# vladiant/CascadeClassifier

Measured on AMD Instinct MI355X. Metric: detection Mwindows/sec (1080p, haarcascade_frontalface) + achieved HBM GB/s, higher is better.
Workload: dtype i32+f32 (f64 stage sums)

## Files before the change

### cascadeclassifier_amd/csrc/cc_eval_kernel.inc

```

#define CC_CONST __attribute__((address_space(4)))
template <class T>
__device__ __forceinline__ const T CC_CONST* as_const_table(const T* p) {
  return (const T CC_CONST*)p;
}
template <class T>
__device__ __forceinline__ T load_record(const T CC_CONST* p) {
  static_assert(sizeof(T) % 4 == 0, "table records are dword multiples");
  T out;
  const int CC_CONST* w = (const int CC_CONST*)p;
  int* o = reinterpret_cast<int*>(&out);
#pragma unroll
  for (unsigned i = 0; i < sizeof(T) / 4; i++) o[i] = w[i];
  return out;
}

constexpr int STAGE_ROWS = 12;
template <int STEP, class Geom>
__device__ __forceinline__ void stage_tile(int32_t* lds, const Geom& G, const int32_t* __restrict__ sum,
                                           const ScaleDev& S, int x0, int y0) {
  const int lane = threadIdx.x & 63, wave = __builtin_amdgcn_readfirstlane(threadIdx.x >> 6);
  const int quads = (G.cols + 3) >> 2;
  const bool right_edge = x0 + quads * 4 - 1 > S.w;
  for (int q0 = 0; q0 < quads; q0 += 64) {
// ... 67 lines not shown
  int sq_compact;
  int split_stumps;
  int stop_after;
  unsigned long long* masks;
  size_t mask_frame_words;
  CandRaw* cands;
  int* cand_count;
  int cand_cap;
  int32_t* dbg_codes;
  double* dbg_sums;
  unsigned long long* stamps;
};
constexpr int STAMP_SLOTS = 40;

struct LdsReader {
  const int32_t* b;
  __device__ __forceinline__ int operator()(int ofs) const { return b[ofs]; }
};
struct GlobalReader {
  const int32_t* g;
  unsigned org;
  int pitch;
  __device__ __forceinline__ int operator()(int p) const { return g[org + (unsigned)((p >> 16) * pitch + (p & 0xffff))]; }
};
template <class R>
__device__ __forceinline__ double stump_vote(const R& rd, const HaarStumpDev& sp, float vnf) {
  const int r0 = rd(sp.ofs[0][0]) - rd(sp.ofs[0][1]) - rd(sp.ofs[0][2]) + rd(sp.ofs[0][3]);
  const int r1 = rd(sp.ofs[1][0]) - rd(sp.ofs[1][1]) - rd(sp.ofs[1][2]) + rd(sp.ofs[1][3]);
  float v = sp.w[0] * (float)r0 + sp.w[1] * (float)r1;
  if (sp.nrect == 3) {
    const int r2 = rd(sp.ofs[2][0]) - rd(sp.ofs[2][1]) - rd(sp.ofs[2][2]) + rd(sp.ofs[2][3]);
    v += sp.w[2] * (float)r2;
  }
  v *= vnf;
  return (double)(v < sp.thr ? sp.left : sp.right);
}
template <class R>
__device__ __forceinline__ double stump_vote(const R& rd, const HaarStumpDev CC_CONST* spp, float vnf) {
  return stump_vote(rd, load_record(spp), vnf);
}

struct Lds16Reader {
  const unsigned short* h;
  __device__ __forceinline__ int operator()(int ofs) const { return (int)h[ofs]; }
};
template <bool M16, class R>
__device__ __forceinline__ float lbp_vote_f(const R& rd, const LbpStumpDev& sp) {
  int p[16];
#pragma unroll
  for (int j = 0; j < 16; j++) p[j] = rd(sp.ofs[j]);
  auto cell = [&](int a, int b, int c2, int d) {
    const int v = p[a] - p[b] - p[c2] + p[d];
    return M16 ? (v & 0xffff) : v;
  };
  const int c = cell(5, 6, 9, 10);
  const bool b7 = cell(0, 1, 4, 5) >= c, b6 = cell(1, 2, 5, 6) >= c, b5 = cell(2, 3, 6, 7) >= c;
  const int lo = (cell(6, 7, 10, 11) >= c ? 16 : 0) | (cell(10, 11, 14, 15) >= c ? 8 : 0) | (cell(9, 10, 13, 14) >= c ? 4 : 0) |
                 (cell(8, 9, 12, 13) >= c ? 2 : 0) | (cell(4, 5, 8, 9) >= c ? 1 : 0);
  const int l0 = b5 ? sp.subset[1] : sp.subset[0], l1 = b5 ? sp.subset[3] : sp.subset[2], l2 = b5 ? sp.subset[5] : sp.subset[4],
            l3 = b5 ? sp.subset[7] : sp.subset[6];
  const int m0 = b6 ? l1 : l0, m1 = b6 ? l3 : l2;
  const unsigned w = (unsigned)(b7 ? m1 : m0);
  return ((w >> lo) & 1u) ? sp.left : sp.right;
}

template <class R>
__device__ __forceinline__ double stump_vote(const R& rd, const LbpStumpDev CC_CONST* sp, float) {
  int p[16];
#pragma unroll
  for (int j = 0; j < 16; j++) p[j] = rd(sp->ofs[j]);
  const int c = p[5] - p[6] - p[9] + p[10];
  const int lbp = (p[0] - p[1] - p[4] + p[5] >= c ? 128 : 0) | (p[1] - p[2] - p[5] + p[6] >= c ? 64 : 0) |
                  (p[2] - p[3] - p[6] + p[7] >= c ? 32 : 0) | (p[6] - p[7] - p[10] + p[11] >= c ? 16 : 0) |
                  (p[10] - p[11] - p[14] + p[15] >= c ? 8 : 0) | (p[9] - p[10] - p[13] + p[14] >= c ? 4 : 0) |
                  (p[8] - p[9] - p[12] + p[13] >= c ? 2 : 0) | (p[4] - p[5] - p[8] + p[9] >= c ? 1 : 0);
  const int word = sp->subset[lbp >> 5];
  return (double)((word & (1 << (lbp & 31))) ? sp->left : sp->right);
}

__device__ __forceinline__ double tree_vote(const int32_t* b, const HaarNodeDev* __restrict__ nodes, int root, int leaf0,
                                            const float* __restrict__ leaves, float vnf) {
  int idx = 0;
  do {
    const HaarNodeDev* n = nodes + root + idx;
    const int r0 = b[n->ofs[0][0]] - b[n->ofs[0][1]] - b[n->ofs[0][2]] + b[n->ofs[0][3]];
    const int r1 = b[n->ofs[1][0]] - b[n->ofs[1][1]] - b[n->ofs[1][2]] + b[n->ofs[1][3]];
    float v = n->w[0] * (float)r0 + n->w[1] * (float)r1;
    if (n->nrect == 3) v += n->w[2] * (float)(b[n->ofs[2][0]] - b[n->ofs[2][1]] - b[n->ofs[2][2]] + b[n->ofs[2][3]]);
    v *= vnf;
    idx = v < n->thr ? n->left : n->right;
  } while (idx > 0);
  return (double)leaves[leaf0 - idx];
}
__device__ __forceinline__ double tree_vote(const int32_t* b, const LbpNodeDev* __restrict__ nodes, int root, int leaf0,
                                            const float* __restrict__ leaves, float) {
  int idx = 0;
  do {
    const LbpNodeDev* n = nodes + root + idx;
    int p[16];
#pragma unroll
    for (int j = 0; j < 16; j++) p[j] = b[n->ofs[j]];
    const int c = p[5] - p[6] - p[9] + p[10];
    const int lbp = (p[0] - p[1] - p[4] + p[5] >= c ? 128 : 0) | (p[1] - p[2] - p[5] + p[6] >= c ? 64 : 0) |
                    (p[2] - p[3] - p[6] + p[7] >= c ? 32 : 0) | (p[6] - p[7] - p[10] + p[11] >= c ? 16 : 0) |
                    (p[10] - p[11] - p[14] + p[15] >= c ? 8 : 0) | (p[9] - p[10] - p[13] + p[14] >= c ? 4 : 0) |
                    (p[8] - p[9] - p[12] + p[13] >= c ? 2 : 0) | (p[4] - p[5] - p[8] + p[9] >= c ? 1 : 0);
    idx = (n->subset[lbp >> 5] & (1 << (lbp & 31))) ? n->left : n->right;
  } while (idx > 0);
  return (double)leaves[leaf0 - idx];
}

template <int CTRL, int ROW_MASK>
__device__ __forceinline__ int dpp_i32(int v) {
  return __builtin_amdgcn_update_dpp(0, v, CTRL, ROW_MASK, 0xF, false);
}
__device__ __forceinline__ int wave_max_u32(int v) {
  v = max(v, dpp_i32<0xB1, 0xF>(v));
  v = max(v, dpp_i32<0x4E, 0xF>(v));
  v = max(v, dpp_i32<0x141, 0xF>(v));
  v = max(v, dpp_i32<0x140, 0xF>(v));
  v = max(v, dpp_i32<0x142, 0xA>(v));
  v = max(v, dpp_i32<0x143, 0xC>(v));
  return __builtin_amdgcn_readlane(v, 63);
}
__device__ __forceinline__ int wave_sum_u32(int v) {
  v += dpp_i32<0xB1, 0xF>(v);
  v += dpp_i32<0x4E, 0xF>(v);
  v += dpp_i32<0x141, 0xF>(v);
  v += dpp_i32<0x140, 0xF>(v);
  v += dpp_i32<0x142, 0xA>(v);
  v += dpp_i32<0x143, 0xC>(v);
  return __builtin_amdgcn_readlane(v, 63);
}

__device__ __forceinline__ float inv_sqrt_as_float(double nf) {
#ifndef CC_EXACT_SLOW_VNF
  double y = __builtin_amdgcn_rsq(nf);
#pragma unroll
  for (int it = 0; it < 2; it++) {
    const double e = __builtin_fma(-(nf * y), y, 1.0);
    y = __builtin_fma(0.5 * y, e, y);
  }
  const unsigned below = (unsigned)(unsigned long long)__double_as_longlong(y) & 0x1fffffffu;
  if (__builtin_expect(below - 0x0ffffc00u > 0x800u, 1)) return (float)y;
#endif
  return (float)(1. / sqrt(nf));
}

#ifdef CC_SPEC_STAGES
template <int STEP>
__device__ __forceinline__ double spec_stage(int st, int p_lo, int p_hi, const int32_t* b, float vnf);
template <int STEP>
__device__ __forceinline__ void spec_stage0_x2(const int32_t* ba, const int32_t* bb, float vnfa, float vnfb, double& acc_a, double& acc_b);
#endif

template <bool C, class A, class B>
struct cc_select {
  using type = A;
};
template <class A, class B>
struct cc_select<false, A, B> {
  using type = B;
};

template <int STEP, bool HAAR, bool TREES>
__device__ __forceinline__ void eval_tile(const EvalArgs& A, int32_t* lds, const int4 T, const ScaleDev& S) {
  using Stump = typename cc_select<HAAR, HaarStumpDev, LbpStumpDev>::type;
  using Node = typename cc_select<HAAR, HaarNodeDev, LbpNodeDev>::type;
  const Node* __restrict__ nodes = reinterpret_cast<const Node*>(STEP == 2 ? A.nodes2 : A.nodes1);
#ifdef CC_SPEC_W0
  constexpr int W0 = CC_SPEC_W0, H0 = CC_SPEC_H0;
#else
  const int W0 = A.W0, H0 = A.H0;
#endif
#ifdef CC_SPEC_TILE16
  constexpr bool G16 = STEP == 2 && !TREES;
#else
  constexpr bool G16 = false;
#endif
  using Geom = typename cc_select<G16, TileGeom16, TileGeom<STEP>>::type;
  const Geom G(W0, H0);
  double* s_part = reinterpret_cast<double*>(lds + tile_words_padded(G.words()) * ((HAAR && A.tilt_chan >= 0) ? 2 : 1));
  float* s_vnf = reinterpret_cast<float*>(s_part + PART_DOUBLES);
  unsigned short* s_q = reinterpret_cast<unsigned short*>(s_vnf + (HAAR ? TILE_Y * VNF_PITCH : 0));
  int* s_cnt = reinterpret_cast<int*>(s_q + 2 * TILE_WINDOWS);
  const int frame = blockIdx.y;
  const int32_t* sum = A.integ + ((size_t)frame * A.nchan + 0) * A.int_frame_elems + S.int_ofs;
  const int lane = threadIdx.x & 63, wave = __builtin_amdgcn_readfirstlane(threadIdx.x >> 6);
  const int gx0 = T.y * TILE_X, gy0 = T.z * TILE_Y;
  const Stump CC_CONST* stumps = as_const_table(reinterpret_cast<const Stump*>(G16 ? A.gstumps : STEP == 2 ? A.stumps2 : A.stumps1));
  const int CC_CONST* stage_first = as_const_table(A.stage_first);
  const int CC_CONST* stage_ntrees = as_const_table(A.stage_ntrees);
  const float CC_CONST* stage_thr = as_const_table(A.stage_thr);
  const bool dbg = A.dbg_codes != nullptr && frame == 0;
  auto stamp = [&](int slot) {
    if (A.stamps && threadIdx.x == 0)
      A.stamps[((size_t)blockIdx.y * gridDim.x + blockIdx.x) * STAMP_SLOTS + slot] = __builtin_amdgcn_s_memtime();
  };
  stamp(0);

  unsigned sq_raw[WIN_PER_THREAD][4];
#pragma unroll
  for (int k = 0; k < WIN_PER_THREAD; k++) {
    sq_raw[k][0] = sq_raw[k][1] = sq_raw[k][2] = sq_raw[k][3] = 0;
    if (HAAR) {
      const int gx = min(gx0 + lane, S.nx - 1), gy = min(gy0 + wave * WIN_PER_THREAD + k, S.ny - 1);
      {
        const unsigned* sq = reinterpret_cast<const unsigned*>(A.integ + ((size_t)frame * A.nchan + 1) * A.int_frame_elems + S.int_ofs);
        const int nrx = W0 - 2, nry = H0 - 2;
        size_t q0;
        int dx;
        if (STEP == 2 && A.sq_compact) {
          q0 = (size_t)(gy * 2 + 1) * S.pitchI + gx;
          dx = nrx >> 1;
        } else {
          q0 = (size_t)(gy * STEP + 1) * S.pitchI + (gx * STEP + 1);
          dx = nrx;
        }
        sq_raw[k][0] = sq[q0];
        sq_raw[k][1] = sq[q0 + dx];
        sq_raw[k][2] = sq[q0 + (size_t)nry * S.pitchI];
        sq_raw[k][3] = sq[q0 + (size_t)nry * S.pitchI + dx];
      }
    }
  }
#ifdef CC_PRIO_STAGE
  __builtin_amdgcn_s_setprio(CC_PRIO_STAGE);
#endif
  stage_tile<STEP>(lds, G, sum, S, gx0 * STEP, gy0 * STEP);
  if (HAAR && A.tilt_chan >= 0)
    stage_tile<STEP>(lds + tile_words_padded(G.words()), G,
                     A.integ + ((size_t)frame * A.nchan + A.tilt_chan) * A.int_frame_elems + S.int_ofs, S, gx0 * STEP, gy0 * STEP);
  if (threadIdx.x < 3 * 32) s_cnt[threadIdx.x] = 0;
  unsigned valsq_pre[WIN_PER_THREAD];
#pragma unroll
  for (int k = 0; k < WIN_PER_THREAD; k++) valsq_pre[k] = sq_raw[k][0] - sq_raw[k][1] - sq_raw[k][2] + sq_raw[k][3];
  __syncthreads();
#ifdef CC_PRIO_STAGE
  __builtin_amdgcn_s_setprio(0);
#endif
  stamp(1);

  if (A.stop_after == -2) return;
  auto window_base = [&](int id) { return ((id >> 6) * STEP) * G.row_stride + (id & 63); };
  auto table_reader = [&](int id) {
    if constexpr (G16)
      return GlobalReader{sum, (unsigned)((gy0 + (id >> 6)) * STEP) * (unsigned)S.pitchI + (unsigned)((gx0 + (id & 63)) * STEP), S.pitchI};
    else
      return LdsReader{lds + window_base(id)};
  };
  auto report = [&](int id, int code, double last) {
    const size_t o = (size_t)S.win_ofs + (size_t)(gy0 + (id >> 6)) * S.nx + (gx0 + (id & 63));
    A.dbg_codes[o] = code;
    if (A.dbg_sums) A.dbg_sums[o] = last;
  };
  auto emit_candidate = [&](int id, double last_sum) {
    const int slot = atomicAdd(A.cand_count, 1);
    if (slot < A.cand_cap) A.cands[slot] = CandRaw{frame, T.x, gx0 + (id & 63), gy0 + (id >> 6), last_sum};
  };
  const int skew = (STEP * G.row_stride) & 31;
  auto win_class = [&](int id) { return ((id & 63) + skew * (id >> 6)) & 31; };
  auto vnf_slot = [&](int id) { return (id >> 6) * (TILE_X + skew) + (id & 63); };
  auto enqueue = [&](bool pass, int id, int g) {
    if (g >= A.dense_from) {
      const unsigned long long m = __ballot(pass);
      int first = 0;
      if (lane == 0 && m) first = atomicAdd(&s_cnt[(g % 3) * 32], __builtin_popcountll(m));
      first = __builtin_amdgcn_readfirstlane(first);
      if (pass) s_q[(g & 1) * TILE_WINDOWS + first + __builtin_amdgcn_mbcnt_hi((unsigned)(m >> 32), __builtin_amdgcn_mbcnt_lo((unsigned)m, 0))] = (unsigned short)id;
    } else if (pass) {
      const int c = win_class(id);
      const int row = atomicAdd(&s_cnt[(g % 3) * 32 + c], 1);
      s_q[(g & 1) * TILE_WINDOWS + row * 32 + c] = (unsigned short)id;
    }
  };

  const int CC_CONST* group_first = as_const_table(A.group_first);
  auto stage_sum = [&](int s, int id, const int32_t* b, float vnf, bool want) -> double {
    double acc = 0.;
    const int first = stage_first[s], nt = stage_ntrees[s];
    if constexpr (TREES) {
      for (int j = 0; j < nt; j++) {
        const int root = as_const_table(A.tree_root)[first + j], leaf0 = as_const_table(A.tree_leaf0)[first + j];
        if (want) acc += tree_vote(b, nodes, root, leaf0, A.leaves, vnf);
      }
    } else {
#ifdef CC_SPEC_STAGES
      if (s < CC_SPEC_STAGES) return spec_stage<STEP>(s, 0, SPEC_PARTS, b, vnf);
#endif
      const auto rd = table_reader(id);
      if constexpr (HAAR) {
        Stump cur = load_record(stumps + first);
        for (int j = 0; j < nt; j++) {
          const Stump nxt = load_record(stumps + first + min(j + 1, nt - 1));
          acc += stump_vote(rd, cur, vnf);
          cur = nxt;
        }
      } else {
        for (int j = 0; j < nt; j++) acc += stump_vote(rd, stumps + first + j, vnf);
      }
    }
    return acc;
  };

  if constexpr (!HAAR && !TREES && WIN_PER_THREAD > 2) {
    const int gx = gx0 + lane;
    const double thr0 = (double)stage_thr[0];
    const int nt0 = stage_ntrees[0];
#pragma unroll 1
    for (int k = 0; k < WIN_PER_THREAD; k++) {
      const int ly = wave * WIN_PER_THREAD + k;
      const int gy = gy0 + ly;
      const int id = ly * 64 + lane;
      const int32_t* b = lds + (ly * STEP) * G.row_stride + lane;
      const bool alive = gx < S.nx && gy < S.ny;
      double acc = 0.;
      if (__any(alive)) {
#ifdef CC_SPEC_STAGES
        acc = spec_stage<STEP>(0, 0, SPEC_PARTS, b, 1.f);
#else
        for (int i = 0; i < nt0; i++) acc += stump_vote(LdsReader{b}, stumps + i, 1.f);
#endif
      }
      (void)nt0;
      bool pass = alive && !(acc < thr0);
      const bool rej0 = alive && !pass;
      const unsigned long long m = __ballot(rej0);
      if (lane == 0 && gy < S.ny) A.masks[(size_t)frame * A.mask_frame_words + S.mask_ofs + (size_t)gy * S.nxw + T.y] = m;
      if (dbg && rej0) report(id, 0, acc);
      if (!dbg && A.early_skip) {
        const unsigned long long lower = (1ull << lane) - 1ull;
        const unsigned long long zeros_below = ~m & lower;
        int run;
        bool known;
        if (zeros_below) {
          run = lane - 1 - (63 - __clzll((long long)zeros_below));
          known = true;
        } else {
          run = lane;
          known = T.y == 0;
        }
        if (known && (run & 1)) pass = false;
      }
      if (A.nstages == 1) {
        if (pass) {
          emit_candidate(id, acc);
          if (dbg) report(id, 1, acc);
        }
      } else
        enqueue(pass, id, 1);
    }
  } else {
    int base[WIN_PER_THREAD];
    float vnf[WIN_PER_THREAD];
    bool alive[WIN_PER_THREAD];
    const int gx = gx0 + lane;
#pragma unroll
    for (int k = 0; k < WIN_PER_THREAD; k++) {
      const int ly = wave * WIN_PER_THREAD + k;
      const int gy = gy0 + ly;
      base[k] = (ly * STEP) * G.row_stride + lane;
      vnf[k] = 1.f;
      alive[k] = gx < S.nx && gy < S.ny;
      if (HAAR) {
        const bool in_grid = alive[k];
        alive[k] = false;
        if (in_grid) {
          const int nrx = W0 - 2, nry = H0 - 2;
          const double area = (double)(nrx * nry);
          const int32_t* b = lds + base[k];
          int valsum;
          if constexpr (G16) {
            const unsigned short* h = reinterpret_cast<const unsigned short*>(b);
            const int hx = nrx >> 1;
            const unsigned a0 = h[G.at(1, 1)], a1 = h[G.at(1, 1 + hx)], a2 = h[G.at(1, 1 + nrx)];
            const unsigned c0 = h[G.at(1 + nry, 1)], c1 = h[G.at(1 + nry, 1 + hx)], c2 = h[G.at(1 + nry, 1 + nrx)];
            valsum = (int)(((a0 - a1 - c0 + c1) & 0xffffu) + ((a1 - a2 - c1 + c2) & 0xffffu));
          } else
            valsum = b[G.at(1, 1)] - b[G.at(1, 1 + nrx)] - b[G.at(1 + nry, 1)] + b[G.at(1 + nry, 1 + nrx)];
          const unsigned valsq = valsq_pre[k];
          double nf = area * (double)valsq - (double)valsum * (double)valsum;
          if (nf > 0.) {
            vnf[k] = inv_sqrt_as_float(nf);
            alive[k] = area * (double)vnf[k] < 1e-1;
          }
          if (dbg && !alive[k]) report(ly * 64 + lane, -1, 0.0);
        }
      }
    }
    if (A.stop_after == -3) {
      float sink = 0;
#pragma unroll
      for (int k = 0; k < WIN_PER_THREAD; k++) sink += alive[k] ? vnf[k] : 0.f;
      if (HAAR && sink == 12345.f) s_vnf[0] = sink;
      return;
    }
    bool any_mine = false;
    double acc[WIN_PER_THREAD];
#pragma unroll
    for (int k = 0; k < WIN_PER_THREAD; k++) {
      any_mine |= alive[k];
      acc[k] = 0.;
    }
    if (__any(any_mine)) {
      const int nt = stage_ntrees[0];
      if constexpr (TREES) {
        for (int i = 0; i < nt; i++) {
          const int root = as_const_table(A.tree_root)[i], leaf0 = as_const_table(A.tree_leaf0)[i];
#pragma unroll
          for (int k = 0; k < WIN_PER_THREAD; k++)
            if (alive[k]) acc[k] += tree_vote(lds + base[k], nodes, root, leaf0, A.leaves, vnf[k]);
        }
      } else if constexpr (HAAR) {
#ifdef CC_SPEC_STAGES
        if constexpr (WIN_PER_THREAD == 2) {
          spec_stage0_x2<STEP>(lds + base[0], lds + base[1], vnf[0], vnf[1], acc[0], acc[1]);
        } else {
#pragma unroll
          for (int k = 0; k < WIN_PER_THREAD; k++) acc[k] = spec_stage<STEP>(0, 0, SPEC_PARTS, lds + base[k], vnf[k]);
        }
#else
        Stump cur = load_record(stumps);
        for (int i = 0; i < nt; i++) {
          const Stump nxt = load_record(stumps + min(i + 1, nt - 1));
#pragma unroll
          for (int k = 0; k < WIN_PER_THREAD; k++) acc[k] += stump_vote(LdsReader{lds + base[k]}, cur, vnf[k]);
          cur = nxt;
        }
#endif
      } else {
#ifdef CC_SPEC_STAGES
        if constexpr (WIN_PER_THREAD == 2) {
          spec_stage0_x2<STEP>(lds + base[0], lds + base[1], vnf[0], vnf[1], acc[0], acc[1]);
        } else {
#pragma unroll
          for (int k = 0; k < WIN_PER_THREAD; k++) acc[k] = spec_stage<STEP>(0, 0, SPEC_PARTS, lds + base[k], vnf[k]);
        }
#else
        for (int i = 0; i < nt; i++) {
#pragma unroll
          for (int k = 0; k < WIN_PER_THREAD; k++) acc[k] += stump_vote(LdsReader{lds + base[k]}, stumps + i, vnf[k]);
        }
#endif
      }
    }
    const double thr = (double)stage_thr[0];
    bool pass_k[WIN_PER_THREAD];
#pragma unroll
    for (int k = 0; k < WIN_PER_THREAD; k++) {
      const int ly = wave * WIN_PER_THREAD + k;
      const int gy = gy0 + ly;
      const int id = ly * 64 + lane;
      bool pass = alive[k] && !(acc[k] < thr);
      const bool rej0 = alive[k] && !pass;
      const unsigned long long m = __ballot(rej0);
      if (lane == 0 && gy < S.ny) A.masks[(size_t)frame * A.mask_frame_words + S.mask_ofs + (size_t)gy * S.nxw + T.y] = m;
      if (dbg && rej0) report(id, 0, acc[k]);
      if (!dbg && A.early_skip) {
        const unsigned long long lower = (1ull << lane) - 1ull;
        const unsigned long long zeros_below = ~m & lower;
        int run;
        bool known;
        if (zeros_below) {
          run = lane - 1 - (63 - __clzll((long long)zeros_below));
          known = true;
        } else {
          run = lane;
          known = T.y == 0;
        }
        if (known && (run & 1)) pass = false;
      }
      pass_k[k] = pass;
    }
#pragma unroll
    for (int k = 0; k < WIN_PER_THREAD; k++) {
      const int id = (wave * WIN_PER_THREAD + k) * 64 + lane;
      const bool pass = pass_k[k];
      if (A.nstages == 1) {
        if (pass) {
          emit_candidate(id, acc[k]);
          if (dbg) report(id, 1, acc[k]);
        }
      } else {
        if (HAAR && pass) s_vnf[vnf_slot(id)] = vnf[k];
        enqueue(pass, id, 1);
      }
    }
  }

  stamp(2);
#ifdef CC_PRIO_LATE
  __builtin_amdgcn_s_setprio(CC_PRIO_LATE);
#endif
  const int half = lane >> 5, cls = lane & 31;
  int st = 1;
  int qg = 1;
  int n = 0, rows = 0, my_rows = 0;
  for (; qg < A.ngroups; qg++) {
    st = group_first[qg];
    const int st_end = group_first[qg + 1];
    if (A.stop_after >= 0 && st > A.stop_after) return;
    __syncthreads();
    if (qg >= A.dense_from) {
      n = min(s_cnt[(qg % 3) * 32], TILE_WINDOWS);
// ... 288 lines not shown
```

### cascadeclassifier_amd/csrc/cc_spec.hip

```cpp
#include <hip/hip_runtime.h>

#include <algorithm>
#include <array>
#include <cmath>
#include <cstdlib>
#include <cstring>
#include <map>
#include <mutex>

#include <dlfcn.h>
#include <sys/stat.h>
#include <unistd.h>

#include "cc_detect_internal.h"

namespace ccamd {

#include "build/cc_eval_kernel_src.h"

struct SpecStump {
  std::string loads;
  std::string decls;
  std::string compute;
  double base = 0.;
  long long base_q = 0;
};

static const char* spec_stage_inline_attr() {
  const char* e = std::getenv("CCAMD_SPEC_NOINLINE");
  return (e && std::atoi(e) != 0) ? "__noinline__" : "__forceinline__";
}

static void spec_emit_stage(std::string& o, const std::vector<SpecStump>& st, int depth, bool parts, const std::vector<std::string>& accs,
                            bool fixed_point = false) {
  const int nt = (int)st.size();
  static const char* kSB = "      __builtin_amdgcn_sched_barrier(0);\n";
  for (const SpecStump& t : st) o += "      " + t.decls + "\n";
  const int P = parts ? SPEC_PARTS : 1;
  char buf[128];
  int prev_nonempty = -1;
  for (int k = 0; k < P; k++) {
    const int e0 = (int)((long long)k * nt / P), e1 = (int)((long long)(k + 1) * nt / P);
    if (e0 == e1) continue;
    if (parts)
      snprintf(buf, sizeof(buf), "      if (p_lo > %d && p_lo <= %d) {\n", prev_nonempty, k);
    else
      snprintf(buf, sizeof(buf), "      {\n");
    prev_nonempty = k;
    o += buf;
    for (int i = e0; i < std::min(e0 + depth, nt); i++) o += "      " + st[(size_t)i].loads + "\n" + kSB;
    o += "      }\n";
    if (parts) {
      snprintf(buf, sizeof(buf), "      if (p_lo <= %d && %d < p_hi) {\n", k, k);
      o += buf;
    } else
      o += "      {\n";
    {
      double base = 0.;
      unsigned base_q = 0;
      for (int i = e0; i < e1; i++) {
        base += st[(size_t)i].base;
        base_q += (unsigned)st[(size_t)i].base_q;
      }
      char lit[64];
      if (fixed_point)
        snprintf(lit, sizeof(lit), "%uu", base_q);
      else
        snprintf(lit, sizeof(lit), "%a", base);
      if (fixed_point ? base_q != 0 : base != 0.)
        for (const std::string& a : accs) o += "      " + a + " += " + lit + ";\n";
    }
    for (int i = e0; i < e1; i++) {
      if (depth > 0 && i + depth < nt) o += "      " + st[(size_t)(i + depth)].loads + "\n" + kSB;
      if (depth == 0) o += "      " + st[(size_t)i].loads + "\n";
      o += "      " + st[(size_t)i].compute + "\n" + kSB;
    }
    o += "      }\n";
  }
}

static std::string spec_stage_source_lbp(const Cascade& m, int n_stages, bool tile16);

static std::vector<std::array<int, 4>> pieces16(int x, int y, int w, int h) {
  std::vector<std::array<int, 4>> out;
  const bool along_x = w >= h;
  const int len = along_x ? w : h;
  for (int k = 1; k <= std::max(len, 1); k++) {
    out.clear();
    bool ok = true;
    for (int i = 0; i < k; i++) {
      const int a = (int)((long long)i * len / k), b = (int)((long long)(i + 1) * len / k);
      if (a == b) continue;
      const std::array<int, 4> pc = along_x ? std::array<int, 4>{x + a, y, b - a, h} : std::array<int, 4>{x, y + a, w, b - a};
      ok = ok && fits16((long long)pc[2] * pc[3]);
      out.push_back(pc);
    }
    if (ok) return out;
  }
  return {};
}

static bool tile16_eligible(const Cascade& m, int n_stages) {
  if (m.max_nodes_per_tree > 1) return false;
  const int total = (int)m.stage_ntrees.size();
  n_stages = std::min<int>(n_stages, total);
  const char* on = std::getenv("CCAMD_SPEC_TILE16");
  if (on ? std::atoi(on) == 0 : !(m.feature_type == CC_FEATURE_LBP && n_stages == total)) return false;
  if (m.feature_type == CC_FEATURE_HAAR) {
    if (m.has_tilted) return false;
    const int nrx = m.win_w - 2, nry = m.win_h - 2;
    if (nrx < 2 || !fits16((long long)(nrx - (nrx >> 1)) * nry)) return false;
    if (!fits16(std::max(m.win_w, m.win_h))) return false;
    return true;
  }
  for (int s = 0; s < n_stages; s++)
    for (int i = 0; i < m.stage_ntrees[(size_t)s]; i++) {
      const int32_t* r = &m.lbp_rects[(size_t)m.stump_feature[(size_t)m.stage_first[(size_t)s] + i] * 4];
      if (!fits16((long long)r[2] * r[3])) return false;
    }
  return true;
}

static std::string spec_stage_source(const Cascade& m, int n_stages, int tmode) {
  const CNumericLocale c_numbers;
  if (m.feature_type == CC_FEATURE_LBP) return spec_stage_source_lbp(m, n_stages, tmode == TILE_16);
  std::vector<HaarStumpDev> t[2];
  build_haar_stumps<1>(m, t[0]);
  build_haar_stumps<2>(m, t[1]);
  const TileGeom16 G16(m.win_w, m.win_h);
  n_stages = std::min<int>(n_stages, (int)m.stage_ntrees.size());
  const int depth = 2;
  const bool delta_form = stage_sums_order_independent(m, 4.0);
  std::string o;
  char buf[512];
  auto hexf = [&](float v) {
    snprintf(buf, sizeof(buf), "%af", (double)v);
    return std::string(buf);
  };
  auto stage_quantum = [&](int s, double& q) {
    int emin = INT32_MAX;
    double mag = 0;
    for (int i = 0; i < m.stage_ntrees[(size_t)s]; i++) {
      const size_t k = (size_t)m.stage_first[(size_t)s] + i;
      const float l = m.stump_left[k], r = m.stump_right[k];
      mag += std::max(std::fabs((double)l), std::fabs((double)r));
      for (float v : {l, r})
        if (v != 0.0f) {
          int e;
          std::frexp(v, &e);
          emin = std::min(emin, e);
        }
    }
    if (emin == INT32_MAX) return false;
    q = std::ldexp(1.0, emin - 24);
    return mag / q < 2147483647.0;
  };
  std::function<std::string(const HaarStumpDev&, const std::string&, double, SpecStump&)> vote_text;
  auto stump = [&](const HaarStumpDev& d, int stump_index, int local, const std::string& win, double fixed_q, bool h16,
                   const std::map<int, std::string>* reuse = nullptr, std::map<int, std::string>* vars_out = nullptr) {
    const int fi = m.stump_feature[(size_t)stump_index];
    const std::string tile_ptr = (h16 ? "h" : "b") + win;
    bool int_ok = true;
    double bound = 0;
    for (int j = 0; j < d.nrect; j++) {
      const float w = d.w[j];
      const int32_t* r = &m.haar_rects[(size_t)fi * 12 + j * 4];
      if (w != std::nearbyint(w) || std::fabs(w) > 64.f) int_ok = false;
      bound += std::fabs((double)w) * 255.0 * (double)r[2] * (double)r[3] * (m.haar_tilted[(size_t)fi] ? 2.0 : 1.0);
    }
    if (bound >= 16777216.0) int_ok = false;
    SpecStump out;
    std::map<int, std::string> var;
    auto var_of = [&](int ofs) {
      auto it = var.find(ofs);
      if (it != var.end()) return it->second;
      if (reuse) {
        auto r = reuse->find(ofs);
        if (r != reuse->end()) return var[ofs] = r->second;
      }
      snprintf(buf, sizeof(buf), "x%d_%d%s", local, (int)var.size(), win.c_str());
      const std::string name = buf;
      var[ofs] = name;
      out.decls += (out.decls.empty() ? "unsigned " : ", ") + name;
      snprintf(buf, sizeof(buf), "%s = (unsigned)%s[%d]; ", name.c_str(), tile_ptr.c_str(), ofs);
      out.loads += buf;
      return name;
    };
    std::string e = "{ float v = ";
    if (h16) {
      long long vmin = 0, vmax = 0;
      if (int_ok) {
        std::vector<int> net((size_t)(m.win_w + 1) * (size_t)(m.win_h + 1), 0);
        for (int j = 0; j < d.nrect; j++) {
          const int32_t* r = &m.haar_rects[(size_t)fi * 12 + j * 4];
          for (int yy = r[1]; yy < r[1] + r[3]; yy++)
            for (int xx = r[0]; xx < r[0] + r[2]; xx++) net[(size_t)yy * (size_t)(m.win_w + 1) + (size_t)xx] += (int)d.w[j];
        }
        for (int v : net) (v > 0 ? vmax : vmin) += 255LL * v;
      }
      if (int_ok && vmin >= -32768 && vmax <= 32767) {
        std::map<int, int> coef;
        static const int sign[4] = {1, -1, -1, 1};
        for (int j = 0; j < d.nrect; j++) {
          const int32_t* r = &m.haar_rects[(size_t)fi * 12 + j * 4];
          const int o4[4] = {G16.at(r[1], r[0]), G16.at(r[1], r[0] + r[2]), G16.at(r[1] + r[3], r[0]), G16.at(r[1] + r[3], r[0] + r[2])};
          for (int k = 0; k < 4; k++) coef[o4[k]] += sign[k] * (int)d.w[j];
        }
        std::map<int, std::vector<int>> by_coef;
        for (auto& kv : coef)
          if (kv.second) by_coef[std::abs(kv.second)].push_back(kv.second > 0 ? kv.first + 1 : -(kv.first + 1));
        std::string tt;
        for (auto& g : by_coef) {
          std::string grp;
          for (int so : g.second) {
            grp += so > 0 ? (grp.empty() ? "" : " + ") : " - ";
            grp += var_of(std::abs(so) - 1);
          }
          if (grp.rfind(" - ", 0) == 0) grp = "0u" + grp;
          snprintf(buf, sizeof(buf), "%s%du * (", tt.empty() ? "" : " + ", g.first);
          tt += buf + grp + ")";
        }
        if (tt.empty()) tt = "0u";
        e += "(float)(int)(short)(" + tt + ")";
      } else {
        std::string terms_int, terms_float;
        for (int j = 0; j < d.nrect; j++) {
          const int32_t* r = &m.haar_rects[(size_t)fi * 12 + j * 4];
          std::string rj;
          for (const auto& pc : pieces16(r[0], r[1], r[2], r[3])) {
            const std::string a = var_of(G16.at(pc[1], pc[0])), b2 = var_of(G16.at(pc[1], pc[0] + pc[2])), c = var_of(G16.at(pc[1] + pc[3], pc[0])),
                              dd = var_of(G16.at(pc[1] + pc[3], pc[0] + pc[2]));
            rj += std::string(rj.empty() ? "" : " + ") + "((" + a + " - " + b2 + " - " + c + " + " + dd + ") & 0xffffu)";
          }
          if (rj.empty()) rj = "0u";
          snprintf(buf, sizeof(buf), "%s%d * (int)(", j ? " + " : "", (int)d.w[j]);
          terms_int += buf + rj + ")";
          terms_float += std::string(j ? " + " : "") + hexf(d.w[j]) + " * (float)(int)(" + rj + ")";
        }
        e += int_ok ? "(float)(" + terms_int + ")" : terms_float;
      }
    } else if (int_ok) {
      std::map<int, int> coef;
      static const int sign[4] = {1, -1, -1, 1};
      for (int j = 0; j < d.nrect; j++)
        for (int k = 0; k < 4; k++) coef[d.ofs[j][k]] += sign[k] * (int)d.w[j];
      std::map<int, std::vector<int>> by_coef;
      for (auto& kv : coef)
        if (kv.second) by_coef[std::abs(kv.second)].push_back(kv.second > 0 ? kv.first + 1 : -(kv.first + 1));
      std::string tt;
      for (auto& g : by_coef) {
        std::string grp;
        for (int so : g.second) {
          grp += so > 0 ? (grp.empty() ? "" : " + ") : " - ";
          grp += var_of(std::abs(so) - 1);
        }
        if (grp.rfind(" - ", 0) == 0) grp = "0u" + grp;
        snprintf(buf, sizeof(buf), "%s%du * (", tt.empty() ? "" : " + ", g.first);
        tt += buf + grp + ")";
      }
      if (tt.empty()) tt = "0u";
      e += "(float)(int)(" + tt + ")";
    } else {
      for (int j = 0; j < d.nrect; j++) {
        const std::string a = var_of(d.ofs[j][0]), b2 = var_of(d.ofs[j][1]), c = var_of(d.ofs[j][2]), dd = var_of(d.ofs[j][3]);
        e += std::string(j ? " + " : "") + hexf(d.w[j]) + " * (float)(int)(" + a + " - " + b2 + " - " + c + " + " + dd + ")";
      }
    }
    if (out.decls.empty()) out.decls = "";
    else out.decls += ";";
    out.compute += e + vote_text(d, win, fixed_q, out);
    if (vars_out) *vars_out = var;
    return out;
  };
  const bool share_corners = !std::getenv("CCAMD_SPEC_NO_SHARE");
  int share_window = 1;
  if (const char* e = std::getenv("CCAMD_SPEC_SHARE_WINDOW")) share_window = std::max(1, std::min(8, std::atoi(e)));
  auto corner_set = [&](const HaarStumpDev& d) {
    std::map<int, int> coef;
    static const int sign[4] = {1, -1, -1, 1};
    for (int j = 0; j < d.nrect; j++)
      for (int k = 0; k < 4; k++) coef[d.ofs[j][k]] += sign[k];
    std::vector<int> v;
    for (auto& kv : coef) v.push_back(kv.first);
    return v;
  };
  auto sharing_order = [&](int s, int step) {
    const int nt = m.stage_ntrees[(size_t)s], f0 = m.stage_first[(size_t)s];
    std::vector<std::vector<int>> pts((size_t)nt);
    for (int i = 0; i < nt; i++) pts[(size_t)i] = corner_set(t[step - 1][(size_t)f0 + i]);
    auto shared_with = [&](int i, const std::vector<int>& recent) {
      int n = 0;
      for (int o : pts[(size_t)i]) n += std::binary_search(recent.begin(), recent.end(), o) ? 1 : 0;
      return n;
    };
    auto part_start = [&](int n) {
      for (int k = 0; k < SPEC_PARTS; k++)
        if (n == (int)((long long)k * nt / SPEC_PARTS)) return true;
      return false;
    };
    std::vector<int> best_order;
    int best_total = -1;
    for (int start = 0; start < nt; start++) {
      std::vector<int> order{start};
      std::vector<char> used((size_t)nt, 0);
      used[(size_t)start] = 1;
      int total = 0;
      for (int n = 1; n < nt; n++) {
        std::vector<int> recent;
        for (int k = 1; k <= share_window && n - k >= 0; k++) {
          const std::vector<int>& q = pts[(size_t)order[(size_t)(n - k)]];
          recent.insert(recent.end(), q.begin(), q.end());
        }
        std::sort(recent.begin(), recent.end());
        int best = -1, best_shared = -1;
        for (int i = 0; i < nt; i++) {
          if (used[(size_t)i]) continue;
          const int sh = shared_with(i, recent);
          if (sh > best_shared) {
            best_shared = sh;
            best = i;
          }
        }
        used[(size_t)best] = 1;
        order.push_back(best);
        if (!part_start(n)) total += best_shared;
      }
      if (total > best_total) {
        best_total = total;
        best_order.swap(order);
      }
    }
    return best_order;
  };
  vote_text = [&](const HaarStumpDev& d, const std::string& win, double fixed_q, SpecStump& out) -> std::string {
    if (delta_form && fixed_q > 0.) {
      char delta[64];
      const long long lq = (long long)std::llround((double)d.left / fixed_q), rq = (long long)std::llround((double)d.right / fixed_q);
      snprintf(delta, sizeof(delta), "0x%08x", (unsigned)(lq - rq));
      char vote[512];
      unsigned thr_bits;
      std::memcpy(&thr_bits, &d.thr, 4);
      snprintf(vote, sizeof(vote),
               "; v *= vnf%s; { unsigned long long sx; asm volatile(\"s_mov_b64 %%1, exec\\n\\tv_cmpx_gt_f32_e32 0x%08x, %%2\\n\\tv_add_u32_e32 %%0, %s, %%0\\n\\ts_mov_b64 exec, %%1\" "
               ": \"+v\"(ai%s), \"=&s\"(sx) : \"v\"(v) : \"vcc\"); } }",
               win.c_str(), thr_bits, delta, win.c_str());
      out.base = (double)d.right;
      out.base_q = rq;
      return vote;
    }
    if (delta_form) {
      char delta[64];
      snprintf(delta, sizeof(delta), "%a", (double)d.left - (double)d.right);
      out.base = (double)d.right;
      return "; v *= vnf" + win + "; acc" + win + " += (v < " + hexf(d.thr) + " ? " + delta + " : 0.); }";
    }
    return "; v *= vnf" + win + "; acc" + win + " += (double)(v < " + hexf(d.thr) + " ? " + hexf(d.left) + " : " + hexf(d.right) + "); }";
  };
  for (int step = 1; step <= 2; step++) {
    snprintf(buf, sizeof(buf),
             "template <>\n__device__ %s double spec_stage<%d>(int st, int p_lo, int p_hi, const int32_t* b, float vnf) {\n", spec_stage_inline_attr(), step);
    o += buf;
    const bool h16 = tmode == TILE_16 && step == 2;
    if (h16) o += "  const unsigned short* h = reinterpret_cast<const unsigned short*>(b);\n";
    o += "  double acc = 0.;\n  switch (st) {\n";
    for (int s = 0; s < n_stages; s++) {
      snprintf(buf, sizeof(buf), "    case %d: {\n", s);
      o += buf;
      std::vector<SpecStump> st;
      double q = 0.;
      const bool fixed = delta_form && stage_quantum(s, q);
      if (fixed && share_corners) {
        const int nt = m.stage_ntrees[(size_t)s];
        const std::vector<int> order = sharing_order(s, step);
        std::vector<std::map<int, std::string>> hist;
        for (int n = 0; n < nt; n++) {
          for (int k = 0; k < SPEC_PARTS; k++)
            if (n == (int)((long long)k * nt / SPEC_PARTS)) hist.clear();
          std::map<int, std::string> recent, cur;
          for (int k = 0; k < share_window && k < (int)hist.size(); k++)
            for (auto& kv : hist[hist.size() - 1 - (size_t)k]) recent.insert(kv);
          const int i = order[(size_t)n];
          st.push_back(stump(t[step - 1][(size_t)m.stage_first[(size_t)s] + i], m.stage_first[(size_t)s] + i, i, "", q, h16, &recent, &cur));
          hist.push_back(cur);
        }
      } else
      for (int i = 0; i < m.stage_ntrees[(size_t)s]; i++)
        st.push_back(stump(t[step - 1][(size_t)m.stage_first[(size_t)s] + i], m.stage_first[(size_t)s] + i, i, "", fixed ? q : 0., h16));
      if (fixed) {
        o += "      unsigned ai = 0u;\n";
        spec_emit_stage(o, st, depth, true, {"ai"}, true);
        snprintf(buf, sizeof(buf), "      acc = (double)(int)ai * %a;\n", q);
        o += buf;
      } else
        spec_emit_stage(o, st, depth, true, {"acc"});
      o += "    } break;\n";
    }
    o += "    default: break;\n  }\n  return acc;\n}\n";
    snprintf(buf, sizeof(buf),
             "template <>\n__device__ __forceinline__ void spec_stage0_x2<%d>(const int32_t* ba, const int32_t* bb, float vnfa, float vnfb, double& "
             "acc_a, double& acc_b) {\n  double acca = 0., accb = 0.;\n  {\n",
             step);
    o += buf;
    if (h16)
      o += "  const unsigned short* ha = reinterpret_cast<const unsigned short*>(ba);\n  const unsigned short* hb = reinterpret_cast<const unsigned short*>(bb);\n";
    {
      std::vector<SpecStump> st;
      double q = 0.;
      const bool fixed = delta_form && stage_quantum(0, q);
      for (int i = 0; i < m.stage_ntrees[0]; i++) {
        const HaarStumpDev& d = t[step - 1][(size_t)m.stage_first[0] + i];
        SpecStump a = stump(d, m.stage_first[0] + i, i, "a", fixed ? q : 0., h16), b2 = stump(d, m.stage_first[0] + i, i, "b", fixed ? q : 0., h16);
        st.push_back(SpecStump{a.loads + b2.loads, a.decls + " " + b2.decls, a.compute + " " + b2.compute, a.base, a.base_q});
      }
      if (fixed) {
        o += "      unsigned aia = 0u, aib = 0u;\n";
        spec_emit_stage(o, st, depth, false, {"aia", "aib"}, true);
        snprintf(buf, sizeof(buf), "      acca = (double)(int)aia * %a;\n      accb = (double)(int)aib * %a;\n", q, q);
        o += buf;
      } else
        spec_emit_stage(o, st, depth, false, {"acca", "accb"});
    }
    o += "  }\n  acc_a = acca;\n  acc_b = accb;\n}\n";
  }
  return o;
}

static std::string spec_stage_source_lbp(const Cascade& m, int n_stages, bool tile16) {
  std::vector<LbpStumpDev> t[2];
  build_lbp_stumps<1>(m, t[0]);
  if (tile16)
    build_lbp_stumps16(m, t[1]);
  else
    build_lbp_stumps<2>(m, t[1]);
  n_stages = std::min<int>(n_stages, (int)m.stage_ntrees.size());
  const int depth = 0;
  std::string o;
  char buf[1024];
  auto hexf = [&](float v) {
    char b2[64];
    snprintf(b2, sizeof(b2), "%af", (double)v);
    return std::string(b2);
  };
  auto stump = [&](const LbpStumpDev& d, int local, const std::string& win, bool h16) {
    SpecStump out;
    std::string P[16];
    for (int k = 0; k < 16; k++) {
      snprintf(buf, sizeof(buf), "p%d_%d%s", local, k, win.c_str());
      P[k] = buf;
      out.decls += (k ? ", " : "int ") + P[k];
      snprintf(buf, sizeof(buf), "%s = %s%s[%d]; ", P[k].c_str(), h16 ? "h" : "b", win.c_str(), d.ofs[k]);
      out.loads += buf;
    }
    out.decls += ";";
    std::string diffs = "const int ";
    bool firstd = true;
    for (int k = 0; k < 15; k++) {
      if (k % 4 == 3) continue;
      snprintf(buf, sizeof(buf), "%sh%d_%d%s = %s - %s", firstd ? "" : ", ", local, k, win.c_str(), P[k].c_str(), P[k + 1].c_str());
      diffs += buf;
      firstd = false;
    }
    diffs += "; ";
    auto cell = [&](int a, int , int c, int ) {
      char hb[96];
      snprintf(hb, sizeof(hb), "h%d_%d%s - h%d_%d%s", local, a, win.c_str(), local, c, win.c_str());
      const std::string v = hb;
      return h16 ? "((" + v + ") & 0xffff)" : v;
    };
    const int* w = d.subset;
    std::string t = "{ " + diffs + "const int c = " + cell(5, 6, 9, 10) + "; const bool b7 = " + cell(0, 1, 4, 5) + " >= c, b6 = " + cell(1, 2, 5, 6) +
                    " >= c, b5 = " + cell(2, 3, 6, 7) + " >= c; const int lo = (" + cell(6, 7, 10, 11) + " >= c ? 16 : 0) | (" +
                    cell(10, 11, 14, 15) + " >= c ? 8 : 0) | (" + cell(9, 10, 13, 14) + " >= c ? 4 : 0) | (" + cell(8, 9, 12, 13) +
                    " >= c ? 2 : 0) | (" + cell(4, 5, 8, 9) + " >= c ? 1 : 0); ";
    snprintf(buf, sizeof(buf),
             "const unsigned l0 = b5 ? 0x%08xu : 0x%08xu, l1 = b5 ? 0x%08xu : 0x%08xu, l2 = b5 ? 0x%08xu : 0x%08xu, l3 = b5 ? 0x%08xu : 0x%08xu; "
             "const unsigned m0 = b6 ? l1 : l0, m1 = b6 ? l3 : l2; const unsigned sw = b7 ? m1 : m0; "
             "acc%s += (double)(((sw >> lo) & 1u) ? %s : %s); }",
             (unsigned)w[1], (unsigned)w[0], (unsigned)w[3], (unsigned)w[2], (unsigned)w[5], (unsigned)w[4], (unsigned)w[7], (unsigned)w[6],
             win.c_str(), hexf(d.left).c_str(), hexf(d.right).c_str());
    out.compute = t + buf;
    return out;
  };
  for (int step = 1; step <= 2; step++) {
    snprintf(buf, sizeof(buf),
             "template <>\n__device__ %s double spec_stage<%d>(int st, int p_lo, int p_hi, const int32_t* b, float vnf) {\n", spec_stage_inline_attr(), step);
    o += buf;
    const bool h16 = tile16 && step == 2;
    if (h16) o += "  const unsigned short* h = reinterpret_cast<const unsigned short*>(b);\n";
    o += "  double acc = 0.;\n  switch (st) {\n";
    for (int s = 0; s < n_stages; s++) {
      snprintf(buf, sizeof(buf), "    case %d: {\n", s);
      o += buf;
      std::vector<SpecStump> st;
      for (int i = 0; i < m.stage_ntrees[(size_t)s]; i++) {
        const int idx = m.stage_first[(size_t)s] + i;
        st.push_back(stump(t[step - 1][(size_t)idx], i, "", h16));
      }
      spec_emit_stage(o, st, depth, true, {"acc"});
      o += "    } break;\n";
    }
    o += "    default: break;\n  }\n  return acc;\n}\n";
    snprintf(buf, sizeof(buf),
             "template <>\n__device__ __forceinline__ void spec_stage0_x2<%d>(const int32_t* ba, const int32_t* bb, float vnfa, float vnfb, double& "
             "acc_a, double& acc_b) {\n  double acca = 0., accb = 0.;\n  {\n",
             step);
    o += buf;
    if (h16)
      o += "  const unsigned short* ha = reinterpret_cast<const unsigned short*>(ba);\n  const unsigned short* hb = reinterpret_cast<const unsigned short*>(bb);\n";
    {
      std::vector<SpecStump> st;
      for (int i = 0; i < m.stage_ntrees[0]; i++) {
        const int idx = m.stage_first[0] + i;
        SpecStump a = stump(t[step - 1][(size_t)idx], i, "a", h16), b2 = stump(t[step - 1][(size_t)idx], i, "b", h16);
        st.push_back(SpecStump{a.loads + b2.loads, a.decls + " " + b2.decls, a.compute + " " + b2.compute});
      }
      spec_emit_stage(o, st, depth, false, {"acca", "accb"});
    }
    o += "  }\n  acc_a = acca;\n  acc_b = accb;\n}\n";
  }
  return o;
}

struct HipRtcApi {
  void* lib = nullptr;
  int (*create)(void**, const char*, const char*, int, const char* const*, const char* const*) = nullptr;
  int (*compile)(void*, int, const char* const*) = nullptr;
  int (*log_size)(void*, size_t*) = nullptr;
  int (*log)(void*, char*) = nullptr;
  int (*code_size)(void*, size_t*) = nullptr;
  int (*code)(void*, char*) = nullptr;
  int (*destroy)(void**) = nullptr;
  int (*version)(int*, int*) = nullptr;
  bool ok() const { return create && compile && log_size && log && code_size && code && destroy; }
};

static const HipRtcApi& hiprtc_api() {
  static HipRtcApi api;
  static std::once_flag once;
  std::call_once(once, [] {
    for (const char* name : {"libhiprtc.so.7", "libhiprtc.so", "/opt/rocm/lib/libhiprtc.so"}) {
      api.lib = dlopen(name, RTLD_NOW | RTLD_LOCAL);
      if (api.lib) break;
    }
    if (!api.lib) return;
    auto sym = [&](const char* n) { return dlsym(api.lib, n); };
    api.create = reinterpret_cast<decltype(api.create)>(sym("hiprtcCreateProgram"));
    api.compile = reinterpret_cast<decltype(api.compile)>(sym("hiprtcCompileProgram"));
    api.log_size = reinterpret_cast<decltype(api.log_size)>(sym("hiprtcGetProgramLogSize"));
    api.log = reinterpret_cast<decltype(api.log)>(sym("hiprtcGetProgramLog"));
    api.code_size = reinterpret_cast<decltype(api.code_size)>(sym("hiprtcGetCodeSize"));
    api.code = reinterpret_cast<decltype(api.code)>(sym("hiprtcGetCode"));
    api.destroy = reinterpret_cast<decltype(api.destroy)>(sym("hiprtcDestroyProgram"));
    api.version = reinterpret_cast<decltype(api.version)>(sym("hiprtcVersion"));
  });
  return api;
}

static const char kSpecPrelude[] =
    "typedef signed char int8_t;\ntypedef unsigned char uint8_t;\ntypedef short int16_t;\ntypedef unsigned short uint16_t;\n"
    "typedef int int32_t;\ntypedef unsigned int uint32_t;\ntypedef long long int64_t;\ntypedef unsigned long long uint64_t;\n";

struct SpecModulePlan {
  int only_step, tile_y;
};
static std::vector<SpecModulePlan> spec_modules(const Cascade& m, int tmode) {
  auto valid = [&](int ty) { return ty >= EVAL_WAVES && ty <= 32 && ty % EVAL_WAVES == 0; };
  auto env_rows = [&](const char* name, int dflt) {
    const char* e = std::getenv(name);
    const int v = e ? std::atoi(e) : dflt;
    return valid(v) ? v : dflt;
  };
  if (m.has_tilted) return {{0, TILE_Y}};
  const bool lbp16 = m.feature_type == CC_FEATURE_LBP && tmode == TILE_16;
  const bool haar32 = tmode == TILE_32 && m.feature_type == CC_FEATURE_HAAR;
  const bool rows_given = std::getenv("CCAMD_SPEC_TILE_Y") != nullptr;
// ... 185 lines not shown
```

Before: 19090.

## Map adjacent window pairs to lanes and load stage-0 corners as 8-byte LDS words

Adds a dense-pairs mode for STEP=2 Haar tiles. Each lane now handles two horizontally adjacent windows (lanes split into two row halves), so the corner fetches for both windows come from shared 8-byte LDS loads. A specialised generated stage-0 evaluator unpacks the paired words, and the rejection masks are re-interleaved with bit spreading before storing. This is meant to halve LDS load instructions in the variance and stage-0 paths, at the cost of extra unpack and mask-shuffle ALU work and a different lane-to-window mapping that can affect bank conflicts.

```diff
diff --git a/cascadeclassifier_amd/csrc/cc_eval_kernel.inc b/cascadeclassifier_amd/csrc/cc_eval_kernel.inc
--- a/cascadeclassifier_amd/csrc/cc_eval_kernel.inc
+++ b/cascadeclassifier_amd/csrc/cc_eval_kernel.inc
@@ -243,6 +243,32 @@
 __device__ __forceinline__ double spec_stage(int st, int p_lo, int p_hi, const int32_t* b, float vnf);
 template <int STEP>
 __device__ __forceinline__ void spec_stage0_x2(const int32_t* ba, const int32_t* bb, float vnfa, float vnfb, double& acc_a, double& acc_b);
+using cc_int2 = int __attribute__((ext_vector_type(2)));
+__device__ __forceinline__ cc_int2 lds_word8(const int32_t* p) {
+  return *(const volatile __attribute__((address_space(3))) cc_int2*)p;
+}
+__device__ __forceinline__ void lds_pair(const int32_t* bp, int o, int& wa, int& wb) {
+  if (o & 1) {
+    const cc_int2 p = lds_word8(bp + o - 1), q = lds_word8(bp + o + 1);
+    wa = p.y;
+    wb = q.x;
+  } else {
+    const cc_int2 p = lds_word8(bp + o);
+    wa = p.x;
+    wb = p.y;
+  }
+}
+__device__ __forceinline__ unsigned long long spread_bits32(unsigned v) {
+  unsigned long long x = v;
+  x = (x | (x << 16)) & 0x0000ffff0000ffffull;
+  x = (x | (x << 8)) & 0x00ff00ff00ff00ffull;
+  x = (x | (x << 4)) & 0x0f0f0f0f0f0f0f0full;
+  x = (x | (x << 2)) & 0x3333333333333333ull;
+  x = (x | (x << 1)) & 0x5555555555555555ull;
+  return x;
+}
+template <int STEP>
+__device__ __forceinline__ void spec_stage0_pair(const int32_t* bp, float vnfa, float vnfb, double& acc_a, double& acc_b);
 #endif
 
 template <bool C, class A, class B>
@@ -279,6 +305,14 @@
   const int32_t* sum = A.integ + ((size_t)frame * A.nchan + 0) * A.int_frame_elems + S.int_ofs;
   const int lane = threadIdx.x & 63, wave = __builtin_amdgcn_readfirstlane(threadIdx.x >> 6);
   const int gx0 = T.y * TILE_X, gy0 = T.z * TILE_Y;
+#ifdef CC_SPEC_DENSE_PAIRS
+  constexpr bool PAIRS = HAAR && !TREES && !G16 && ((CC_SPEC_DENSE_PAIRS >> (STEP - 1)) & 1) != 0;
+#else
+  constexpr bool PAIRS = false;
+#endif
+  constexpr int PAIR_SLOTS = PAIRS ? (WIN_PER_THREAD & ~1) : 0;
+  auto slot_ly = [&](int k) { return wave * WIN_PER_THREAD + (k < PAIR_SLOTS ? (k & ~1) + (lane >> 5) : k); };
+  auto slot_lx = [&](int k) { return k < PAIR_SLOTS ? 2 * (lane & 31) + (k & 1) : lane; };
   const Stump CC_CONST* stumps = as_const_table(reinterpret_cast<const Stump*>(G16 ? A.gstumps : STEP == 2 ? A.stumps2 : A.stumps1));
   const int CC_CONST* stage_first = as_const_table(A.stage_first);
   const int CC_CONST* stage_ntrees = as_const_table(A.stage_ntrees);
@@ -295,7 +329,7 @@
   for (int k = 0; k < WIN_PER_THREAD; k++) {
     sq_raw[k][0] = sq_raw[k][1] = sq_raw[k][2] = sq_raw[k][3] = 0;
     if (HAAR) {
-      const int gx = min(gx0 + lane, S.nx - 1), gy = min(gy0 + wave * WIN_PER_THREAD + k, S.ny - 1);
+      const int gx = min(gx0 + slot_lx(k), S.nx - 1), gy = min(gy0 + slot_ly(k), S.ny - 1);
       {
         const unsigned* sq = reinterpret_cast<const unsigned*>(A.integ + ((size_t)frame * A.nchan + 1) * A.int_frame_elems + S.int_ofs);
         const int nrx = W0 - 2, nry = H0 - 2;
@@ -441,6 +475,118 @@
       } else
         enqueue(pass, id, 1);
     }
+  } else if constexpr (PAIRS) {
+#ifdef CC_SPEC_DENSE_PAIRS
+    int base[WIN_PER_THREAD], valsum[WIN_PER_THREAD];
+    float vnf[WIN_PER_THREAD];
+    bool alive[WIN_PER_THREAD];
+    const int nrx = W0 - 2, nry = H0 - 2;
+    const double area = (double)(nrx * nry);
+    const int vo[4] = {G.at(1, 1), G.at(1, 1 + nrx), G.at(1 + nry, 1), G.at(1 + nry, 1 + nrx)};
+#pragma unroll
+    for (int k = 0; k < WIN_PER_THREAD; k++) base[k] = (slot_ly(k) * STEP) * G.row_stride + slot_lx(k);
+#pragma unroll
+    for (int k = 0; k < PAIR_SLOTS; k += 2) {
+      int ca[4], cb[4];
+#pragma unroll
+      for (int j = 0; j < 4; j++) lds_pair(lds + base[k], vo[j], ca[j], cb[j]);
+      valsum[k] = ca[0] - ca[1] - ca[2] + ca[3];
+      valsum[k + 1] = cb[0] - cb[1] - cb[2] + cb[3];
+    }
+    if constexpr (PAIR_SLOTS < WIN_PER_THREAD) {
+      const int32_t* b = lds + base[WIN_PER_THREAD - 1];
+      valsum[WIN_PER_THREAD - 1] = b[vo[0]] - b[vo[1]] - b[vo[2]] + b[vo[3]];
+    }
+#pragma unroll
+    for (int k = 0; k < WIN_PER_THREAD; k++) {
+      vnf[k] = 1.f;
+      alive[k] = false;
+      if (gx0 + slot_lx(k) < S.nx && gy0 + slot_ly(k) < S.ny) {
+        const double nf = area * (double)valsq_pre[k] - (double)valsum[k] * (double)valsum[k];
+        if (nf > 0.) {
+          vnf[k] = inv_sqrt_as_float(nf);
+          alive[k] = area * (double)vnf[k] < 1e-1;
+        }
+        if (dbg && !alive[k]) report(slot_ly(k) * 64 + slot_lx(k), -1, 0.0);
+      }
+    }
+    if (A.stop_after == -3) {
+      float sink = 0;
+#pragma unroll
+      for (int k = 0; k < WIN_PER_THREAD; k++) sink += alive[k] ? vnf[k] : 0.f;
+      if (sink == 12345.f) s_vnf[0] = sink;
+      return;
+    }
+    bool any_mine = false;
+    double acc[WIN_PER_THREAD];
+#pragma unroll
+    for (int k = 0; k < WIN_PER_THREAD; k++) {
+      any_mine |= alive[k];
+      acc[k] = 0.;
+    }
+    if (__any(any_mine)) {
+#pragma unroll
+      for (int k = 0; k < PAIR_SLOTS; k += 2) spec_stage0_pair<STEP>(lds + base[k], vnf[k], vnf[k + 1], acc[k], acc[k + 1]);
+      if constexpr (PAIR_SLOTS < WIN_PER_THREAD)
+        acc[WIN_PER_THREAD - 1] = spec_stage<STEP>(0, 0, SPEC_PARTS, lds + base[WIN_PER_THREAD - 1], vnf[WIN_PER_THREAD - 1]);
+    }
+    const double thr = (double)stage_thr[0];
+    bool pass_k[WIN_PER_THREAD];
+    auto skipped = [&](unsigned long long m, int col) {
+      const unsigned long long zeros_below = ~m & ((1ull << col) - 1ull);
+      int run;
+      bool known;
+      if (zeros_below) {
+        run = col - 1 - (63 - __clzll((long long)zeros_below));
+        known = true;
+      } else {
+        run = col;
+        known = T.y == 0;
+      }
+      return known && (run & 1);
+    };
+    auto store_mask = [&](int gy, unsigned long long m) {
+      A.masks[(size_t)frame * A.mask_frame_words + S.mask_ofs + (size_t)gy * S.nxw + T.y] = m;
+    };
+#pragma unroll
+    for (int k = 0; k < WIN_PER_THREAD; k++) {
+      pass_k[k] = alive[k] && !(acc[k] < thr);
+      if (dbg && alive[k] && !pass_k[k]) report(slot_ly(k) * 64 + slot_lx(k), 0, acc[k]);
+    }
+#pragma unroll
+    for (int k = 0; k < PAIR_SLOTS; k += 2) {
+      const unsigned long long ma = __ballot(alive[k] && !pass_k[k]), mb = __ballot(alive[k + 1] && !pass_k[k + 1]);
+      const unsigned long long m_first = spread_bits32((unsigned)ma) | (spread_bits32((unsigned)mb) << 1);
+      const unsigned long long m_second = spread_bits32((unsigned)(ma >> 32)) | (spread_bits32((unsigned)(mb >> 32)) << 1);
+      const unsigned long long m = (lane >> 5) ? m_second : m_first;
+      const int gy = gy0 + slot_ly(k);
+      if ((lane & 31) == 0 && gy < S.ny) store_mask(gy, m);
+      if (!dbg && A.early_skip) {
+        if (skipped(m, slot_lx(k))) pass_k[k] = false;
+        if (skipped(m, slot_lx(k + 1))) pass_k[k + 1] = false;
+      }
+    }
+    if constexpr (PAIR_SLOTS < WIN_PER_THREAD) {
+      constexpr int k = WIN_PER_THREAD - 1;
+      const unsigned long long m = __ballot(alive[k] && !pass_k[k]);
+      const int gy = gy0 + slot_ly(k);
+      if (lane == 0 && gy < S.ny) store_mask(gy, m);
+      if (!dbg && A.early_skip && skipped(m, lane)) pass_k[k] = false;
+    }
+#pragma unroll
+    for (int k = 0; k < WIN_PER_THREAD; k++) {
+      const int id = slot_ly(k) * 64 + slot_lx(k);
+      if (A.nstages == 1) {
+        if (pass_k[k]) {
+          emit_candidate(id, acc[k]);
+          if (dbg) report(id, 1, acc[k]);
+        }
+      } else {
+        if (pass_k[k]) s_vnf[vnf_slot(id)] = vnf[k];
+        enqueue(pass_k[k], id, 1);
+      }
+    }
+#endif
   } else {
     int base[WIN_PER_THREAD];
     float vnf[WIN_PER_THREAD];
diff --git a/cascadeclassifier_amd/csrc/cc_spec.hip b/cascadeclassifier_amd/csrc/cc_spec.hip
--- a/cascadeclassifier_amd/csrc/cc_spec.hip
+++ b/cascadeclassifier_amd/csrc/cc_spec.hip
@@ -131,7 +131,13 @@
   n_stages = std::min<int>(n_stages, (int)m.stage_ntrees.size());
   const int depth = 2;
   const bool delta_form = stage_sums_order_independent(m, 4.0);
+  int pairs_mask = (tmode == TILE_32 && !m.has_tilted) ? 2 : 0;
+  if (const char* e = std::getenv("CCAMD_SPEC_DENSE_PAIRS")) pairs_mask = pairs_mask ? (std::atoi(e) & 3) : 0;
+  int pair_depth[2] = {0, 1};
+  for (int s = 0; s < 2; s++)
+    if (const char* e = std::getenv(s ? "CCAMD_SPEC_PAIR_DEPTH2" : "CCAMD_SPEC_PAIR_DEPTH1")) pair_depth[s] = std::max(0, std::min(3, std::atoi(e)));
   std::string o;
+  if (pairs_mask) o += "#define CC_SPEC_DENSE_PAIRS " + std::to_string(pairs_mask) + "\n";
   char buf[512];
   auto hexf = [&](float v) {
     snprintf(buf, sizeof(buf), "%af", (double)v);
@@ -421,6 +427,54 @@
         spec_emit_stage(o, st, depth, false, {"acca", "accb"});
     }
     o += "  }\n  acc_a = acca;\n  acc_b = accb;\n}\n";
+    if (pairs_mask & (1 << (step - 1))) {
+      snprintf(buf, sizeof(buf),
+               "template <>\n__device__ __forceinline__ void spec_stage0_pair<%d>(const int32_t* bp, float vnfa, float vnfb, double& acc_a, double& "
+               "acc_b) {\n  double acca = 0., accb = 0.;\n  {\n",
+               step);
+      o += buf;
+      std::vector<SpecStump> st;
+      double q = 0.;
+      const bool fixed = delta_form && stage_quantum(0, q);
+      for (int i = 0; i < m.stage_ntrees[0]; i++) {
+        const HaarStumpDev& d = t[step - 1][(size_t)m.stage_first[0] + i];
+        std::map<int, std::string> vars;
+        SpecStump a = stump(d, m.stage_first[0] + i, i, "a", fixed ? q : 0., false, nullptr, &vars),
+                  b2 = stump(d, m.stage_first[0] + i, i, "b", fixed ? q : 0., false);
+        std::map<int, std::string> words;
+        auto word_of = [&](int even_ofs) {
+          auto it = words.find(even_ofs);
+          if (it != words.end()) return it->second;
+          char nm[48];
+          snprintf(nm, sizeof(nm), "w%d_%d", i, (int)words.size());
+          return words[even_ofs] = nm;
+        };
+        std::string unpack;
+        for (const auto& kv : vars) {
+          std::string nb = kv.second;
+          nb.back() = 'b';
+          const int ofs = kv.first;
+          if (ofs & 1)
+            unpack += kv.second + " = (unsigned)" + word_of(ofs - 1) + ".y; " + nb + " = (unsigned)" + word_of(ofs + 1) + ".x; ";
+          else
+            unpack += kv.second + " = (unsigned)" + word_of(ofs) + ".x; " + nb + " = (unsigned)" + word_of(ofs) + ".y; ";
+        }
+        std::string loads, wdecls;
+        for (const auto& kv : words) {
+          wdecls += (wdecls.empty() ? "cc_int2 " : ", ") + kv.second;
+          loads += kv.second + " = lds_word8(bp + " + std::to_string(kv.first) + "); ";
+        }
+        st.push_back(SpecStump{loads, wdecls + "; " + a.decls + " " + b2.decls, unpack + a.compute + " " + b2.compute, a.base, a.base_q});
+      }
+      if (fixed) {
+        o += "      unsigned aia = 0u, aib = 0u;\n";
+        spec_emit_stage(o, st, pair_depth[step - 1], false, {"aia", "aib"}, true);
+        snprintf(buf, sizeof(buf), "      acca = (double)(int)aia * %a;\n      accb = (double)(int)aib * %a;\n", q, q);
+        o += buf;
+      } else
+        spec_emit_stage(o, st, pair_depth[step - 1], false, {"acca", "accb"});
+      o += "  }\n  acc_a = acca;\n  acc_b = accb;\n}\n";
+    }
   }
   return o;
 }
```

After: 19020. No clear change (-0.4%).
